# WGLab/DeepMod

Measured on AMD Instinct MI355X. Metric: base-positions/sec (whole node), E. coli 5mC wd21/f7 BiLSTM, higher is better.
Workload: dtype f16x3

## Files before the change

deepmod_amd/csrc/deepmod_hip.hip:

```cpp
#include "kernels.h"

#include <dlfcn.h>
#include <rccl/rccl.h>

#include <algorithm>
#include <cmath>
#include <cstdarg>
#include <cstdint>
#include <cstdio>
#include <cstring>
#include <string>
#include <utility>
#include <thread>
#include <type_traits>
#include <vector>

#include "../../include/deepmod_hip.h"
#include "head.hip.inc"

using dmk::Packed16;
using dmk::Packed32;

namespace {

// ... 292 lines not shown
    return ensure_pack(m->d_wpack16qi, dmk::pack_weights_f16q(m->host_weights.data(), true, m->i8s_q), dmk::f16q_prepare(1));
}


int launch_bilstm(dm_model* m, const float* d_x, long long xstride, int64_t n, float* d_prob, uint8_t* d_cls, const int* d_widx = nullptr) {
    if (n <= 0) return DM_OK;
    hipEvent_t e0 = nullptr, e1 = nullptr;
    if (m->profile) {
        if (m->events_used == m->events.size()) {
            if (m->events.size() >= 4096) {
                int rc = flush_profile(m);
                if (rc) return rc;
            } else {
                hipEvent_t a, b;
                HIP_TRY(hipEventCreate(&a));
                HIP_TRY(hipEventCreate(&b));
                m->events.emplace_back(a, b);
            }
        }
        e0 = m->events[m->events_used].first;
        e1 = m->events[m->events_used].second;
        ++m->events_used;
        HIP_TRY(hipEventRecord(e0, m->stream));
    }
    const int ntiles = int((n + dmk::TILE_M - 1) / dmk::TILE_M);
    {
        int rcp = ensure_plogit(m, ntiles);
        if (rcp) return rcp;
    }
    const long long npad = (long long)ntiles * dmk::TILE_M;
    int grid = std::min(2 * ntiles, m->grid_cap);
    if (2 * ntiles > m->grid_cap) {
        const int rounds = (2 * ntiles + m->grid_cap - 1) / m->grid_cap;
        grid = (2 * ntiles + rounds - 1) / rounds;
    }
    m->last_grid = grid;
    if (m->precision == DM_PREC_F16X3 || m->precision == DM_PREC_F16I8 || m->precision == DM_PREC_F16X3_ROLES) {
        const bool i8 = m->precision == DM_PREC_F16I8;
        const bool q16 = m->precision == DM_PREC_F16X3 && m->f16_q;
        const bool qi8 = i8 && m->f16_q;
#ifdef DM_WITH_F16S
        int rc = qi8 ? ensure_f16qi(m) : i8 ? ensure_f16i8(m) : (q16 ? ensure_f16q(m) : ensure_f16s(m));
#else
        if (!m->f16_q || m->precision == DM_PREC_F16X3_ROLES) return fail(DM_EINVAL, "the 32x32x16 kernels are not part of this build (tools/experiments/f16s: DM_WITH_F16S=1)");
        int rc = qi8 ? ensure_f16qi(m) : ensure_f16q(m);
#endif
        if (rc) return rc;
        dmk::F16Args a;
        a.wpack = qi8 ? m->d_wpack16qi : i8 ? m->d_wpack16i : q16 ? m->d_wpack16q : m->d_wpack16s;
        a.hpack = m->d_wout;
        a.x = d_x;
        a.xstride = xstride;
        a.widx = d_widx;
        a.n = n;
        a.ntiles = ntiles;
        a.plogit = m->d_plogit;
        a.len_shift = m->len_shift;
        a.range_flag = m->d_range_flag + m->range_cur;
        a.i8s = qi8 ? m->i8s_q : i8 ? m->i8s : nullptr;
        if (q16 || qi8) dmk::f16q_launch(qi8 ? 1 : 0, a, grid, m->stream);
#ifdef DM_WITH_F16S
        else dmk::f16s_launch(i8 ? 1 : (m->precision == DM_PREC_F16X3_ROLES ? 2 : 0), a, grid, m->stream);
#endif
    } else {
        dmk::F32Args a;
        a.wpack = m->d_wpack;
        a.bpack = m->d_bpack;
        a.hpack = m->d_hpack;
        a.bout0 = m->bout[0];
        a.bout1 = m->bout[1];
        a.x = d_x;
        a.xstride = xstride;
        a.widx = d_widx;
        a.n = n;
        a.prob = d_prob;
        a.cls = d_cls;
        a.scratch = m->d_scratch;
        a.ntiles = ntiles;
        a.dbg = m->d_dbg;
        a.dir_split = 1;
        a.plogit = m->d_plogit;
        dmk::f32_launch(a, grid, m->stream);
    }
    hipLaunchKernelGGL(lstmhead::head_finish_kernel, dim3(unsigned((n + 255) / 256)), dim3(256), 0, m->stream, m->d_plogit, (long long)n,
                       npad, m->bout[0], m->bout[1], d_prob, d_cls);
    HIP_TRY(hipGetLastError());
    if (m->profile) {
        HIP_TRY(hipEventRecord(e1, m->stream));
        ++m->prof_launches;
        m->prof_windows += n;
    }
    return DM_OK;
}

int range_error(dm_model* m) {
    return fail(DM_ERANGE, "DM_PREC_F16X3: an input feature is outside the representable range (features 0-5: |x| <= 65504, "
                "feature 6: |x| <= 65504 * 2^%d, no NaN); the results of these launches are invalid - repeat them with DM_PREC_F32",
                m->len_shift);
}
bool take_range_slot(dm_model* m, int slot) {
    volatile int* f = reinterpret_cast<volatile int*>(m->range_flag) + slot;
    const bool bad = *f != 0;
    *f = 0;
    return bad;
}
int check_range_all(dm_model* m) {
    if (!m->range_flag) return DM_OK;
    bool bad = take_range_slot(m, m->range_cur);
    for (int i = 0; i < DM_MARKS; ++i)
        if (m->mark_slot[i] >= 0) {
            bad |= take_range_slot(m, m->mark_slot[i]);
            m->slot_free[m->mark_slot[i]] = true;
            m->mark_slot[i] = -1;
        }
    for (int sl : m->range_orphans) {
        bad |= take_range_slot(m, sl);
        m->slot_free[sl] = true;
    }
    m->range_orphans.clear();
    return bad ? range_error(m) : DM_OK;
}
int sync_and_check(dm_model* m) {
    HIP_TRY(hipStreamSynchronize(m->stream));
    return check_range_all(m);
}

int predict_common(dm_model* m, const float* x, long long xstride, int64_t x_floats_total, int64_t n,
                   float* prob, uint8_t* cls, bool windows_materialised) {
    if (!m) return fail(DM_EINVAL, "null model");
    if (n < 0) return fail(DM_EINVAL, "negative window count");
    if (n == 0) return DM_OK;
    if (!x) return fail(DM_EINVAL, "null input");
    HIP_TRY(hipSetDevice(m->device));
    const bool xdev = is_device_ptr(x);
    const bool pdev = prob ? is_device_ptr(prob) : true;
    const bool cdev = cls ? is_device_ptr(cls) : true;
    if (xdev && pdev && cdev) {
        int rc = launch_bilstm(m, x, xstride, n, prob, cls);
        if (rc) return rc;
        if (!m->async) return sync_and_check(m);
        return DM_OK;
    }
    if (!windows_materialised) {
        int rc = ensure_stage(m, x_floats_total);
        if (rc) return rc;
        const float* dx = x;
        if (!xdev) {
            HIP_TRY(hipMemcpyAsync(m->d_x, x, sizeof(float) * x_floats_total, hipMemcpyHostToDevice, m->stream));
            dx = m->d_x;
        }
        for (int64_t off = 0; off < n; off += dm_model::STAGE_WINDOWS) {
            const int64_t cnt = std::min<int64_t>(dm_model::STAGE_WINDOWS, n - off);
            float* dp = prob ? (pdev ? prob + 2 * off : m->d_prob) : nullptr;
            uint8_t* dc = cls ? (cdev ? cls + off : m->d_cls) : nullptr;
            rc = launch_bilstm(m, dx + off * xstride, xstride, cnt, dp, dc);
            if (rc) return rc;
            if (prob && !pdev)
                HIP_TRY(hipMemcpyAsync(prob + 2 * off, m->d_prob, sizeof(float) * 2 * cnt, hipMemcpyDeviceToHost, m->stream));
            if (cls && !cdev) HIP_TRY(hipMemcpyAsync(cls + off, m->d_cls, cnt, hipMemcpyDeviceToHost, m->stream));
            rc = sync_and_check(m);
            if (rc) return rc;
        }
        return DM_OK;
    }
    const int64_t stage_floats = int64_t(dm_model::STAGE_WINDOWS) * DM_WINDOW * DM_NFEAT;
    int rc = ensure_stage(m, stage_floats);
    if (rc) return rc;
    if (!xdev && !m->d_x2) {
// ... 1093 lines not shown
```

deepmod_amd/csrc/kernels.h:

```cpp
#pragma once
#include <hip/hip_runtime.h>

#if defined(DM16Q_ABL_NOCELL) || defined(DM16Q_ABL_NODMA) || defined(DM16Q_ABL_MIX1) || defined(DM16Q_ABL_I8T) || defined(DM16Q_ABL_NOBAR) || defined(DM16Q_ABL_NOVMWAIT) || defined(DM16Q_AINIT) || defined(DM16Q_DEBUG_NOP) ||           \
    defined(DM16Q_NOCHUNK) || defined(DM16Q_NOPN) || defined(DM16Q_LOPACK) || defined(DM16Q_PRE) || defined(DM16Q_SNAKE) || defined(DM16Q_TRANS_COST) ||                     \
    defined(DM16S_ABL_2PROD) || defined(DM16S_ABL_B64) || defined(DM16S_ABL_LO_ONLY) || defined(DM16S_ABL_MFMA16) ||                              \
    defined(DM16S_ABL_MFMA16_PAD) || defined(DM16S_ABL_NOBAR) || defined(DM16S_ABL_NOCELL) || defined(DM16S_ABL_NODMA) ||                          \
    defined(DM16S_ABL_NOLDSA) || defined(DM16S_ADIST) || defined(DM16S_ALO_TRUNC) || defined(DM16S_PRE) || defined(DM_ABL_NOBAR) ||                \
    defined(DM_ABL_NODMA) || defined(DM_ABL_NOEPI) || defined(DM_ABL_NOSEQ) || defined(DM_TIMING) || defined(DM_TRACE) || defined(DM_TRACE2) ||   \
    defined(DM_WLO_TRUNC_ENV) || defined(DM_WLO_TRUNC_DEFAULT) || defined(DM_WITH_F16X3_ROLES) || defined(DM16R_DMA_M) ||                         \
    defined(DM_F16X3_SHAPE_DEFAULT) || defined(DM_WAVES) || defined(DM_MT) || defined(DM_WITH_F16S)
#define DM_ANY_EXPERIMENT_SWITCH 1
#ifndef DM_EXPERIMENT
#error "an ablation / experiment macro is defined without -DDM_EXPERIMENT: timing-only kernels must not be built into the product by a stray -D"
#endif
#else
#define DM_ANY_EXPERIMENT_SWITCH 0
#endif


#if defined(DM_WITH_F16X3_ROLES) && !defined(DM_WITH_F16S)
#error "the roles experiment lives in the translation unit of the 32x32x16 kernels: build it with -DDM_WITH_F16S as well"
#endif

#include <algorithm>
#include <cmath>
#include <cstdint>
#include <cstdlib>
#include <cstring>
#include <vector>

#include "../../include/deepmod_hip.h"

#ifndef DM_F16X3_SHAPE_DEFAULT
#define DM_F16X3_SHAPE_DEFAULT 16
#endif

namespace dmk {

constexpr int TILE_M = 128;

inline float gate_scale(int gc) { return (gc >= 100 && gc < 200) ? 2.8853900817779268f : -1.4426950408889634f; }


struct Packed32 {
    std::vector<float> w, b, h;
    float bout[2];
};

struct Packed16 {
    std::vector<unsigned char> w;
    float max_abs = 0.0f;
    bool finite = true;
    int len_shift = 0;
};

inline int choose_len_shift(const float* flat) {
    float m = 0.0f;
    const float* p = flat;
    for (int d = 0; d < 2; ++d) {
        const float* row = p + size_t(DM_NFEAT - 1) * 400;
        for (int gc = 0; gc < 400; ++gc) m = std::max(m, std::fabs(row[gc] * gate_scale(gc)));
        p += size_t(DM_NFEAT + DM_HIDDEN) * 400 + 400 + 2 * (size_t(2 * DM_HIDDEN) * 400 + 400);
    }
    int k = 10;
    while (k > 0 && !(m * std::ldexp(1.0f, k) <= 32768.0f)) --k;
    return k;
}



struct F16Args {
    const unsigned char* wpack;
    const float* hpack;
    const float* x;
    long long xstride;
    const int* widx;
    long long n;
    int ntiles;
    float* plogit;
    int len_shift;
    int* range_flag;
    const float* i8s;
};
struct F32Args {
    const float *wpack, *bpack, *hpack;
    float bout0, bout1;
    const float* x;
// ... 31 lines not shown
```

deepmod_amd/csrc/lstm_f16q.hip.inc:

```
#ifndef DM16Q_TRANS_COST
#define DM16Q_TRANS_COST 2
#endif
namespace lstm16q {

using lstmc::floatx2;
using lstmc::floatx4;
using lstmc::halfx2;
using lstmc::halfx8;
using lstmc::uintx4;
using lstmc::Params;
using lstmc::ex2;
using lstmc::rcp;
using lstmc::min60;
using lstmc::split_pack;
using lstmc::static_for;
using lstmc::as_h8;

constexpr int HID = 100, NFEAT = 7, WIN = 21, LIVE = 11;
constexpr int NTILE = 13;
constexpr int WAVES = 4, THREADS = 64 * WAVES, TILE_M = 32 * WAVES;
constexpr int KS_L0 = 4, KS_L12 = 7;
constexpr int REC_BYTES = 4096;
constexpr int MIX_BYTES = 2048;
constexpr int TILE_BYTES_L0 = (KS_L0 - 1) * REC_BYTES + 2 * MIX_BYTES, TILE_BYTES_L12 = (KS_L12 - 1) * REC_BYTES + MIX_BYTES;
constexpr int SLOT_BYTES = TILE_BYTES_L12;
constexpr int NSLOT = 2;
constexpr int C2_WAVE_BYTES = NTILE * 1024;
constexpr int C2_LAYER_BYTES = WAVES * C2_WAVE_BYTES;
constexpr size_t LDS_BYTES = size_t(NSLOT) * SLOT_BYTES + C2_LAYER_BYTES;
constexpr size_t LDS_BYTES_I8 = LDS_BYTES + C2_LAYER_BYTES;
constexpr size_t WEIGHT_BYTES_DIR = size_t(NTILE) * (TILE_BYTES_L0 + 2 * TILE_BYTES_L12);
constexpr size_t WEIGHT_BYTES = 2 * WEIGHT_BYTES_DIR;

using lstmc::intx4;
using lstmc::I8_MAGIC;
using lstmc::I8_HI_SCALE;
using lstmc::I8_LO_SCALE;
struct CellPipe {
    float ef[4], ei[4], ej[4], eo[4], t0[4], t1[4];
    unsigned hi01, hi23, lo01, lo23, i01, i23;
    floatx2 fold[2];
    floatx2 kmagic, khi, klo;
    static constexpr int NM = 14;
    template <int PRE, int FMT>
    __device__ static constexpr int nops(int M) {
        constexpr int n[9] = {12, 12, 12, 12, 8, 4, 4, 8, 6};
        if (M == 0) return PRE ? 16 : 0;
        if (M <= 9) return n[M - 1];
        if (M == 10) return FMT >= 1 ? 2 : 0;
        if (M == 11) return 4;
#if defined(DM16Q_LOPACK)
        if (M == 12) return FMT == 2 ? 2 : 0;
#else
        if (M == 12) return FMT != 1 ? 2 : 0;
#endif
        return FMT >= 1 ? 8 : 0;
    }
    template <int M, int J, int FMT = 0>
    __device__ __forceinline__ void op(floatx4 (&g)[4], const intx4 (&gi)[4], const floatx2 (&S)[2], float* c2, const bool only_a) {
        constexpr float K2 = 2.0f * 1.4426950408889634f;
        constexpr int q = J & 3, lv = J >> 2;
#define DM_PIN(X) asm volatile("" : "+v"(X))
        if constexpr (M == 0) {
            constexpr int k = J >> 1, c = k >> 1, pr = k & 1;
            if (only_a && (c & 1)) return;
            if constexpr ((J & 1) == 0) {
                fold[pr] = floatx2{(float)gi[c][2 * pr], (float)gi[c][2 * pr + 1]};
            } else {
                const floatx2 gp = __builtin_elementwise_fma(fold[pr], S[pr], floatx2{g[c][2 * pr], g[c][2 * pr + 1]});
                g[c][2 * pr] = gp[0];
                g[c][2 * pr + 1] = gp[1];
            }
            return;
        }
        if (only_a && (((M <= 8 || M == 11) && (q & 1)) || (M == 9 && lv == 0 && (q & 1)))) return;
        if constexpr (M == 1) {
            if constexpr (lv == 0) { t0[q] = min60(g[q][1]); DM_PIN(t0[q]); }
            else if constexpr (lv == 1) { ef[q] = ex2(g[q][2]); DM_PIN(ef[q]); }
            else { ei[q] = ex2(g[q][0]); DM_PIN(ei[q]); }
        } else if constexpr (M == 2) {
            if constexpr (lv == 0) { ej[q] = ex2(t0[q]); DM_PIN(ej[q]); }
            else if constexpr (lv == 1) { eo[q] = ex2(g[q][3]); DM_PIN(eo[q]); }
            else { ef[q] = 1.0f + ef[q]; DM_PIN(ef[q]); }
        } else if constexpr (M == 3) {
            if constexpr (lv == 0) { ef[q] = rcp(ef[q]); DM_PIN(ef[q]); }
            else if constexpr (lv == 1) { t1[q] = 1.0f + ej[q]; DM_PIN(t1[q]); }
            else { t0[q] = fmaf(ej[q], K2, -K2); DM_PIN(t0[q]); }
        } else if constexpr (M == 4) {
            if constexpr (lv == 0) { ei[q] = fmaf(ei[q], t1[q], t1[q]); DM_PIN(ei[q]); }
            else if constexpr (lv == 1) { eo[q] = 1.0f + eo[q]; DM_PIN(eo[q]); }
            else { ei[q] = rcp(ei[q]); DM_PIN(ei[q]); }
        } else if constexpr (M == 5) {
            if constexpr (lv == 0) { t0[q] = t0[q] * ei[q]; DM_PIN(t0[q]); }
            else { c2[q] = fmaf(c2[q], ef[q], t0[q]); DM_PIN(c2[q]); }
        } else if constexpr (M == 6) {
            { t0[q] = ex2(c2[q]); DM_PIN(t0[q]); }
        } else if constexpr (M == 7) {
            { t1[q] = t0[q] - 1.0f; DM_PIN(t1[q]); }
        } else if constexpr (M == 8) {
            if constexpr (lv == 0) { t0[q] = fmaf(t0[q], eo[q], eo[q]); DM_PIN(t0[q]); }
            else { t0[q] = rcp(t0[q]); DM_PIN(t0[q]); }
        } else if constexpr (M == 9) {
            if constexpr (lv == 0) { t1[q] = t1[q] * t0[q]; DM_PIN(t1[q]); }
            else if constexpr (J == 4) { hi01 = __builtin_bit_cast(unsigned, halfx2{(_Float16)t1[0], (_Float16)t1[1]}); DM_PIN(hi01); }
            else { hi23 = __builtin_bit_cast(unsigned, halfx2{(_Float16)t1[2], (_Float16)t1[3]}); DM_PIN(hi23); }
        } else if constexpr (M == 10) {
            const floatx2 v = __builtin_elementwise_fma(floatx2{t1[2 * J], t1[2 * J + 1]}, khi, kmagic);
            ef[2 * J] = v[0];
            ef[2 * J + 1] = v[1];
        } else if constexpr (M == 11) {
#if defined(DM16Q_LOPACK) && DM16Q_LOPACK == 1
            if constexpr (FMT == 0) {
                if constexpr (q == 0) asm volatile("v_fma_mixlo_f16 %0, %1, -1.0, %2 op_sel:[0,0,0] op_sel_hi:[1,0,0]" : "+v"(lo01) : "v"(hi01), "v"(t1[0]));
// ... 173 lines not shown
    intx4 acci[3][4];
    floatx2 i8s[3][2];
    CellPipe cp;
    float xf[2][2];
    int slot;
};

template <int LAYER, int MM>
__device__ __forceinline__ void c2_load(WaveState& w, const unsigned c2lds, const int tile, float (&row)[4]) {
    if constexpr (LAYER == 2) {
#pragma unroll
        for (int q = 0; q < 4; ++q) row[q] = w.c2reg[tile][q];
    } else if constexpr (LAYER == 1 && MM == 0) {
#pragma unroll
        for (int q = 0; q < 4; ++q) row[q] = w.c1reg[tile][q];
    } else {
        floatx4 v;
        asm volatile("ds_read_b128 %0, %1 offset:%2" : "=v"(v) : "v"(c2lds), "i"(LAYER * C2_LAYER_BYTES));
#pragma unroll
        for (int q = 0; q < 4; ++q) row[q] = v[q];
    }
}
template <int LAYER, int MM>
__device__ __forceinline__ void c2_store(WaveState& w, const unsigned c2lds, const int tile, const float (&row)[4]) {
    if constexpr (LAYER == 2) {
#pragma unroll
        for (int q = 0; q < 4; ++q) w.c2reg[tile][q] = row[q];
    } else if constexpr (LAYER == 1 && MM == 0) {
#pragma unroll
        for (int q = 0; q < 4; ++q) w.c1reg[tile][q] = row[q];
    } else {
        asm volatile("ds_write_b128 %0, %1 offset:%2" :: "v"(c2lds), "v"(floatx4{row[0], row[1], row[2], row[3]}), "i"(LAYER * C2_LAYER_BYTES) : "memory");
    }
}

__device__ __forceinline__ unsigned lo_lo(unsigned a, unsigned b) { return __builtin_amdgcn_perm(b, a, 0x05040100u); }
__device__ __forceinline__ unsigned hi_lo(unsigned a, unsigned b) { return __builtin_amdgcn_alignbit(b, a, 16); }

template <int LAYER, bool FIRST, int MM>
__device__ __forceinline__ void run_stage(const Params& p, WaveState& w, const unsigned lds_base, const unsigned c2_wave, const unsigned char* wdir, const int dir, const int s,
                                          const float* xwin0, const float* xwin1, const int wave_s, const unsigned lane16, const int grp, const unsigned one2) {
    using K = StageKind<LAYER, FIRST>;
    constexpr bool L0 = K::L0;
    constexpr int KS = K::KS;
    constexpr int PREV = (LAYER + 2) % 3;
    constexpr int I8 = (MM == 1 && !(L0 && FIRST)) ? 1 : 0;
    constexpr int PRE = I8;
    constexpr int PPRE = (MM == 1 && !(PREV == 0 && FIRST)) ? 1 : 0;
    constexpr int FMT = MM == 0 ? 0 : (LAYER == 2 ? 2 : 1);
    constexpr size_t LAYER_OFF[3] = {0, size_t(NTILE) * TILE_BYTES_L0, size_t(NTILE) * (TILE_BYTES_L0 + TILE_BYTES_L12)};
    uintx4 (&own)[12] = w.own[LAYER];
    const uintx4 (&inp)[12] = w.own[L0 ? 0 : LAYER - 1];
    const floatx2 (&S)[2] = w.i8s[LAYER];
    const floatx2 (&PS)[2] = w.i8s[PREV];
    uintx4 mx[2], mx2[2];
    unsigned x0p[2] = {0u, 0u}, x1a[2] = {0u, 0u}, x1b[2] = {0u, 0u};
    if constexpr (L0) {
        bool bad = false;
#pragma unroll
        for (int hh = 0; hh < 2; ++hh) {
            float v0 = w.xf[hh][0], v1 = w.xf[hh][1];
            bad |= !(fabsf(v0) <= 65504.0f);
            if (grp < 2) bad |= !(fabsf(v1) <= 65504.0f);
            else {
                const float t = rintf(v1 * p.len_scale);
                bad |= !(fabsf(t) <= 65504.0f);
                v1 = grp == 2 ? v1 - t * p.len_mul : t;
            }
            unsigned xh, xl;
            split_pack(v0, v1, xh, xl);
            x0p[hh] = lo_lo(xh, xl);
            x1a[hh] = __builtin_amdgcn_perm(xh, xh, 0x03020302u);
            x1b[hh] = __builtin_amdgcn_perm(xl, xl, 0x03020302u);
        }
        if (bad) *p.range_flag = 1;
        if (s + 1 < LIVE) {
            const int row = dir == 0 ? s + 1 : WIN - 2 - s;
            const int f1 = 4 + grp < NFEAT ? 4 + grp : NFEAT - 1;
            w.xf[0][0] = xwin0[row * NFEAT + grp]; w.xf[0][1] = xwin0[row * NFEAT + f1];
            w.xf[1][0] = xwin1[row * NFEAT + grp]; w.xf[1][1] = xwin1[row * NFEAT + f1];
        }
    }
    const bool last_stage = LAYER == 2 && s == LIVE - 1;
    static_for<NTILE>([&](auto Tc) {
        constexpr int T = decltype(Tc)::value;
        constexpr int P = T == 0 ? NTILE - 1 : T - 1;
        constexpr int accT = T == NTILE - 1 ? 2 : (T & 1), accP = P == NTILE - 1 ? 2 : (P & 1);
        constexpr bool WITH_B = T < NTILE - 1;
        constexpr int NMF = (WITH_B ? 4 : 2) * (I8 ? 2 : 3);
        float c2row[4];
        if constexpr (T == 0) c2_load<PREV, MM>(w, c2_wave + unsigned(NTILE - 1) * 1024u, NTILE - 1, c2row);
        else c2_load<LAYER, MM>(w, c2_wave + unsigned(P) * 1024u, P, c2row);
        const unsigned a_addr = lds_base + unsigned(w.slot) * SLOT_BYTES + lane16;
#ifdef DM16Q_AINIT
        AQuad a[2] = {};
#else
        AQuad a[2];
#endif
        load_a<K::rec_off(0), WITH_B, K::mixed(0)>(a[0], a_addr);
        if (!(last_stage && T == NTILE - 1)) {
            if constexpr (T + 1 < NTILE) {
                unsigned toff = unsigned(T + 1) * K::TILE_BYTES;
                asm volatile("" : "+s"(toff));
                stage_tile<K::DMA_BYTES>(wdir + (LAYER_OFF[LAYER] + K::DMA_OFF) + toff, lds_base + unsigned(w.slot ^ 1) * SLOT_BYTES + K::DMA_OFF, wave_s, lane16);
            } else {
                using KN = StageKind<(LAYER + 1) % 3, FIRST && LAYER < 2>;
                stage_tile<KN::DMA_BYTES>(wdir + (LAYER_OFF[(LAYER + 1) % 3] + KN::DMA_OFF), lds_base + unsigned(w.slot ^ 1) * SLOT_BYTES + KN::DMA_OFF, wave_s, lane16);
            }
        }
        floatx4 (&d)[4] = w.acc[accT];
        intx4 (&di)[4] = w.acci[accT];
        floatx4 (&g)[4] = w.acc[accP];
        const intx4 (&gi)[4] = w.acci[accP];
        const floatx4 z4 = {0.f, 0.f, 0.f, 0.f};
        const intx4 zi4 = {0, 0, 0, 0};
        constexpr int NCH = DM16Q_PRE + NMF * (KS - 1);
#ifdef DM16Q_NOCHUNK
#define DM_CHUNK(C) do { if constexpr ((C) == NCH - 1) { if constexpr (T == 0) w.cp.template all<PPRE, 0>(g, gi, PS, c2row, true); else w.cp.template all<PRE, FMT>(g, gi, S, c2row, false); } } while (0)
#else
#define DM_CHUNK(C) do { if constexpr (T == 0) w.cp.template chunk<(C), NCH, PPRE, 0>(g, gi, PS, c2row, true); else w.cp.template chunk<(C), NCH, PRE, FMT>(g, gi, S, c2row, false); } while (0)
#endif
        if constexpr (KS > 1) static_for<DM16Q_PRE>([&](auto cc) { DM_CHUNK(decltype(cc)::value); });
        static_for<KS>([&](auto ic) {
            constexpr int i = decltype(ic)::value;
            constexpr int MIXED = K::mixed(i);
            if constexpr (i + 1 < KS) load_a<K::rec_off(i + 1), WITH_B, K::mixed(i + 1)>(a[(i + 1) & 1], a_addr);
            if constexpr (i == KS - 1) {
                if constexpr (KS == 1) {
                    if constexpr (T == 0) w.cp.template all<PPRE, 0>(g, gi, PS, c2row, true);
                    else w.cp.template all<PRE, FMT>(g, gi, S, c2row, false);
                }
#ifdef DM16Q_ABL_NOCELL
                w.cp.hi01 = w.cp.hi23 = 0x2E662E66u; w.cp.lo01 = w.cp.lo23 = 0x0A660A66u;
#endif
                if constexpr (T == 0) {
                    w.m12[PREV][0][0] = lo_lo(w.cp.hi01, w.cp.hi01); w.m12[PREV][0][1] = lo_lo(w.cp.hi01, w.cp.lo01);
                    w.m12[PREV][1][0] = lo_lo(w.cp.hi23, w.cp.hi23); w.m12[PREV][1][1] = lo_lo(w.cp.hi23, w.cp.lo23);
                    c2_store<PREV, MM>(w, c2_wave + unsigned(NTILE - 1) * 1024u, NTILE - 1, c2row);
                } else {
                    constexpr int pt = P >> 2, pr = P & 3;
                    unsigned s01, s23;
                    if constexpr (FMT == 0) { s01 = w.cp.lo01; s23 = w.cp.lo23; }
                    else if constexpr (FMT == 1) { s01 = w.cp.i01; s23 = w.cp.i23; }
                    else { s01 = last_stage ? w.cp.lo01 : w.cp.i01; s23 = last_stage ? w.cp.lo23 : w.cp.i23; }
                    w.nxt[quad(pt, 0, 0)][pr] = w.cp.hi01; w.nxt[quad(pt, 0, 1)][pr] = s01;
                    w.nxt[quad(pt, 1, 0)][pr] = w.cp.hi23; w.nxt[quad(pt, 1, 1)][pr] = s23;
                    c2_store<LAYER, MM>(w, c2_wave + unsigned(P) * 1024u, P, c2row);
                }
            }
            if constexpr (T == 0) {
                static_for<3>([&](auto pc) {
                    constexpr int pt = decltype(pc)::value;
                    if constexpr (KS > 3 ? pt == i : i == 0) {
#pragma unroll
                        for (int e = 0; e < 4; ++e) w.own[PREV][4 * pt + e] = w.nxt[4 * pt + e];
                    }
                });
            }
            if constexpr (MIXED != 0 && T == 0) {
#pragma unroll
                for (int hh = 0; hh < 2; ++hh) {
                    unsigned in_hl;
                    if constexpr (L0) in_hl = x0p[hh];
                    else in_hl = w.m12[LAYER - 1][hh][1];
                    unsigned own_hh = w.m12[LAYER][hh][0], own_hl = w.m12[LAYER][hh][1];
                    asm volatile("" : "+v"(own_hh), "+v"(own_hl), "+v"(in_hl));
                    mx[hh] = uintx4{own_hh, hi_lo(own_hl, in_hl), in_hl, one2};
                    if constexpr (L0) mx2[hh] = uintx4{x1a[hh], x1b[hh], 0u, 0u};
                }
            }
            wait_a<(i + 1 < KS ? a_reads(WITH_B, K::mixed(i + 1 < KS ? i + 1 : i)) : 0)>(a[i & 1]);
            constexpr int C0 = DM16Q_PRE + NMF * i;
#define DM_MF(AOP, BOP, Q, NO)                                                                                              \
            d[Q] = __builtin_amdgcn_mfma_f32_16x16x32_f16(AOP, BOP, (i == 0 && (NO) == 0) ? z4 : d[Q], 0, 0, 0);              \
            asm volatile(DM16Q_AFTER_MFMA : "+v"(d[Q]) : "v"(AOP), "v"(BOP));
#define DM_MI(AOP, BOP, Q)                                                                                                  \
            di[Q] = __builtin_amdgcn_mfma_i32_16x16x64_i8(__builtin_bit_cast(intx4, AOP), __builtin_bit_cast(intx4, BOP), i == 0 ? zi4 : di[Q], 0, 0, 0); \
            asm volatile(DM16Q_AFTER_MFMA : "+v"(di[Q]) : "v"(AOP), "v"(BOP));
#define DM_CELLQ(N_) if constexpr (KS > 1 && i < KS - 1) DM_CHUNK(C0 + (N_))
            if constexpr (MIXED != 0) {
                const halfx8 b0 = as_h8(mx[0]), b1 = as_h8(mx[1]);
                DM_MF(a[i & 1].hiA, b0, 0, 0)
                DM_MF(a[i & 1].hiA, b1, 2, 0)
                if constexpr (WITH_B) { DM_MF(a[i & 1].hiB, b0, 1, 0) DM_MF(a[i & 1].hiB, b1, 3, 0) }
                if constexpr (MIXED == 2) {
                    const halfx8 e0 = as_h8(mx2[0]), e1 = as_h8(mx2[1]);
                    DM_MF(a[i & 1].loA, e0, 0, 1)
                    DM_MF(a[i & 1].loA, e1, 2, 1)
                    if constexpr (WITH_B) { DM_MF(a[i & 1].loB, e0, 1, 1) DM_MF(a[i & 1].loB, e1, 3, 1) }
                }
            } else {
                constexpr int t = K::opnd(i);
                halfx8 bh[2], bl[2];
#pragma unroll
                for (int hh = 0; hh < 2; ++hh) {
                    if constexpr (K::is_own(i)) { bh[hh] = as_h8(own[quad(t, hh, 0)]); bl[hh] = as_h8(own[quad(t, hh, 1)]); }
                    else { bh[hh] = as_h8(inp[quad(t, hh, 0)]); bl[hh] = as_h8(inp[quad(t, hh, 1)]); }
                }
                if constexpr (I8) {
                    DM_MF(a[i & 1].hiA, bh[0], 0, 0) DM_CELLQ(0);
                    DM_MF(a[i & 1].hiA, bh[1], 2, 0) DM_CELLQ(1);
                    if constexpr (WITH_B) { DM_MF(a[i & 1].hiB, bh[0], 1, 0) DM_CELLQ(2); DM_MF(a[i & 1].hiB, bh[1], 3, 0) DM_CELLQ(3); }
                    DM_MI(a[i & 1].loA, bl[0], 0) DM_CELLQ(WITH_B ? 4 : 2);
                    DM_MI(a[i & 1].loA, bl[1], 2) DM_CELLQ(WITH_B ? 5 : 3);
                    if constexpr (WITH_B) { DM_MI(a[i & 1].loB, bl[0], 1) DM_CELLQ(6); DM_MI(a[i & 1].loB, bl[1], 3) DM_CELLQ(7); }
                } else {
#ifdef DM16Q_SNAKE
                DM_MF(a[i & 1].hiA, bh[0], 0, 0) DM_CELLQ(0);
                if constexpr (WITH_B) { DM_MF(a[i & 1].hiB, bh[0], 1, 0) DM_CELLQ(1); DM_MF(a[i & 1].hiB, bh[1], 3, 0) DM_CELLQ(2); }
                DM_MF(a[i & 1].hiA, bh[1], 2, 0) DM_CELLQ(WITH_B ? 3 : 1);
                DM_MF(a[i & 1].loA, bh[1], 2, 1) DM_CELLQ(WITH_B ? 4 : 2);
                if constexpr (WITH_B) { DM_MF(a[i & 1].loB, bh[1], 3, 1) DM_CELLQ(5); DM_MF(a[i & 1].loB, bh[0], 1, 1) DM_CELLQ(6); }
                DM_MF(a[i & 1].loA, bh[0], 0, 1) DM_CELLQ(WITH_B ? 7 : 3);
                DM_MF(a[i & 1].hiA, bl[0], 0, 2) DM_CELLQ(WITH_B ? 8 : 4);
                if constexpr (WITH_B) { DM_MF(a[i & 1].hiB, bl[0], 1, 2) DM_CELLQ(9); DM_MF(a[i & 1].hiB, bl[1], 3, 2) DM_CELLQ(10); }
                DM_MF(a[i & 1].hiA, bl[1], 2, 2) DM_CELLQ(WITH_B ? 11 : 5);
#else
                DM_MF(a[i & 1].hiA, bh[0], 0, 0) DM_CELLQ(0);
                DM_MF(a[i & 1].hiA, bh[1], 2, 0) DM_CELLQ(1);
                if constexpr (WITH_B) { DM_MF(a[i & 1].hiB, bh[0], 1, 0) DM_CELLQ(2); DM_MF(a[i & 1].hiB, bh[1], 3, 0) DM_CELLQ(3); }
#ifdef DM16Q_ABL_I8T
                DM_MI(a[i & 1].loA, bl[0], 0) DM_CELLQ(WITH_B ? 4 : 2); DM_CELLQ(WITH_B ? 5 : 3);
                DM_MI(a[i & 1].loA, bl[1], 2) DM_CELLQ(WITH_B ? 6 : 4); DM_CELLQ(WITH_B ? 7 : 5);
                if constexpr (WITH_B) { DM_MI(a[i & 1].loB, bl[0], 1) DM_CELLQ(8); DM_CELLQ(9); DM_MI(a[i & 1].loB, bl[1], 3) DM_CELLQ(10); DM_CELLQ(11); }
#else
                DM_MF(a[i & 1].loA, bh[0], 0, 1) DM_CELLQ(WITH_B ? 4 : 2);
                DM_MF(a[i & 1].loA, bh[1], 2, 1) DM_CELLQ(WITH_B ? 5 : 3);
                if constexpr (WITH_B) { DM_MF(a[i & 1].loB, bh[0], 1, 1) DM_CELLQ(6); DM_MF(a[i & 1].loB, bh[1], 3, 1) DM_CELLQ(7); }
                DM_MF(a[i & 1].hiA, bl[0], 0, 2) DM_CELLQ(WITH_B ? 8 : 4);
                DM_MF(a[i & 1].hiA, bl[1], 2, 2) DM_CELLQ(WITH_B ? 9 : 5);
                if constexpr (WITH_B) { DM_MF(a[i & 1].hiB, bl[0], 1, 2) DM_CELLQ(10); DM_MF(a[i & 1].hiB, bl[1], 3, 2) DM_CELLQ(11); }
#endif
#endif
                }
            }
#undef DM_MF
#undef DM_MI
#undef DM_CELLQ
        });
#undef DM_CHUNK
#ifndef DM16Q_ABL_NOVMWAIT
        asm volatile("s_waitcnt vmcnt(0)" ::: "memory");
#endif
#ifndef DM16Q_ABL_NOBAR
        __builtin_amdgcn_s_barrier();
#endif
        w.slot ^= 1;
    });
}

template <int MM>
__global__ __launch_bounds__(THREADS, 1) void bilstm_f16q_kernel(const Params p) {
    extern __shared__ __attribute__((aligned(16))) unsigned char lds16q[];
    const int lane = threadIdx.x & 63;
    const int wave = threadIdx.x >> 6;
    const int wave_s = __builtin_amdgcn_readfirstlane(wave);
    const int grp = lane >> 4, n16 = lane & 15;
    const unsigned lane16 = unsigned(lane) * 16u;
    const unsigned lds_base = (unsigned)(size_t)lds16q;
    const unsigned c2_wave = lds_base + unsigned(NSLOT) * SLOT_BYTES + unsigned(wave) * C2_WAVE_BYTES + lane16;
    const unsigned one2 = grp == 0 ? 0x3C003C00u : 0u;
    const int nwork = 2 * p.ntiles;
    for (int work = blockIdx.x; work < nwork; work += gridDim.x) {
        const int tile = work >> 1, dir = work & 1;
        const long long tile0 = (long long)tile * TILE_M;
        const long long w_out = tile0 + wave * 32 + n16;
        long long wi0 = w_out, wi1 = w_out + 16;
        if (wi0 > p.n - 1) wi0 = p.n - 1;
        if (wi1 > p.n - 1) wi1 = p.n - 1;
        const float* xwin0 = p.x + (p.widx ? (long long)p.widx[wi0] : wi0) * p.xstride;
        const float* xwin1 = p.x + (p.widx ? (long long)p.widx[wi1] : wi1) * p.xstride;
        const unsigned char* wdir = p.wpack + size_t(dir) * WEIGHT_BYTES_DIR;

        WaveState w;
#pragma unroll
        for (int l = 0; l < 3; ++l) {
#pragma unroll
            for (int q = 0; q < 12; ++q) w.own[l][q] = uintx4{0u, 0u, 0u, 0u};
#pragma unroll
            for (int hh = 0; hh < 2; ++hh) w.m12[l][hh][0] = w.m12[l][hh][1] = 0u;
        }
#pragma unroll
        for (int q = 0; q < 12; ++q) w.nxt[q] = uintx4{0u, 0u, 0u, 0u};
#pragma unroll
        for (int t = 0; t < NTILE; ++t)
#pragma unroll
            for (int q = 0; q < 4; ++q) w.c2reg[t][q] = w.c1reg[t][q] = 0.0f;
#pragma unroll
        for (int t = 0; t < 3; ++t)
#pragma unroll
            for (int q = 0; q < 4; ++q) w.acc[t][q] = floatx4{0.f, 0.f, 0.f, 0.f};
        w.cp.hi01 = w.cp.hi23 = w.cp.lo01 = w.cp.lo23 = 0u;
        if constexpr (MM == 1) {
#pragma unroll
            for (int t = 0; t < 3; ++t)
#pragma unroll
                for (int q = 0; q < 4; ++q) w.acci[t][q] = intx4{0, 0, 0, 0};
#pragma unroll
            for (int l = 0; l < 3; ++l)
#pragma unroll
                for (int k = 0; k < 2; ++k) w.i8s[l][k] = floatx2{p.i8s[(dir * 3 + l) * 4 + 2 * k], p.i8s[(dir * 3 + l) * 4 + 2 * k + 1]};
            w.cp.kmagic = floatx2{I8_MAGIC, I8_MAGIC};
            w.cp.khi = floatx2{I8_HI_SCALE, I8_HI_SCALE};
            w.cp.klo = floatx2{I8_LO_SCALE, I8_LO_SCALE};
            w.cp.i01 = w.cp.i23 = 0u;
        }
        w.slot = 0;
        __syncthreads();
        {
            const floatx4 z4 = {0.f, 0.f, 0.f, 0.f};
#pragma unroll
            for (int t = 0; t < NTILE; ++t) {
                asm volatile("ds_write_b128 %0, %1" :: "v"(c2_wave + unsigned(t * 1024)), "v"(z4) : "memory");
                if constexpr (MM == 1) asm volatile("ds_write_b128 %0, %1 offset:%2" :: "v"(c2_wave + unsigned(t * 1024)), "v"(z4), "i"(C2_LAYER_BYTES) : "memory");
            }
        }
        {
            using K0 = StageKind<0, true>;
            stage_tile<K0::DMA_BYTES>(wdir + K0::DMA_OFF, lds_base + K0::DMA_OFF, wave_s, lane16);
        }
        {
            const int row = dir == 0 ? 0 : WIN - 1;
            const int f1 = 4 + grp < NFEAT ? 4 + grp : NFEAT - 1;
            w.xf[0][0] = xwin0[row * NFEAT + grp]; w.xf[0][1] = xwin0[row * NFEAT + f1];
            w.xf[1][0] = xwin1[row * NFEAT + grp]; w.xf[1][1] = xwin1[row * NFEAT + f1];
        }
        asm volatile("s_waitcnt vmcnt(0) lgkmcnt(0)" ::: "memory");
        __syncthreads();

#define DM_STAGE(LAYER, FIRST, S_) run_stage<LAYER, FIRST, MM>(p, w, lds_base, c2_wave, wdir, dir, S_, xwin0, xwin1, wave_s, lane16, grp, one2)
        DM_STAGE(0, true, 0);
        DM_STAGE(1, true, 0);
        DM_STAGE(2, true, 0);
        for (int s = 1; s < LIVE; ++s) {
            DM_STAGE(0, false, s);
            DM_STAGE(1, false, s);
            DM_STAGE(2, false, s);
        }
#undef DM_STAGE
        {
            float c2row[4];
#pragma unroll
            for (int q = 0; q < 4; ++q) c2row[q] = w.c2reg[NTILE - 1][q];
            w.cp.template all<MM, 0>(w.acc[2], w.acci[2], w.i8s[2], c2row, true);
            w.m12[2][0][1] = lo_lo(w.cp.hi01, w.cp.lo01);
            w.m12[2][1][1] = lo_lo(w.cp.hi23, w.cp.lo23);
#pragma unroll
            for (int q = 0; q < 12; ++q) w.own[2][q] = w.nxt[q];
        }
#pragma unroll
        for (int hh = 0; hh < 2; ++hh) {
            float hsum0 = 0.0f, hsum1 = 0.0f;
            static_for<NTILE>([&](auto Sc) {
                constexpr int S = decltype(Sc)::value;
                unsigned hi, lo;
                if constexpr (S < 12) { hi = w.own[2][quad(S >> 2, hh, 0)][S & 3]; lo = w.own[2][quad(S >> 2, hh, 1)][S & 3]; }
                else { hi = w.m12[2][hh][1]; lo = w.m12[2][hh][1] >> 16; }
                const halfx2 h2 = __builtin_bit_cast(halfx2, hi), l2 = __builtin_bit_cast(halfx2, lo);
#pragma unroll
                for (int rh = 0; rh < (S < 12 ? 2 : 1); ++rh) {
                    const float h = (float)h2[rh] + (float)l2[rh];
                    const float* wo = p.hpack + (dir * HID + 8 * S + 4 * rh + grp) * 2;
                    hsum0 = fmaf(h, wo[0], hsum0);
                    hsum1 = fmaf(h, wo[1], hsum1);
                }
            });
            hsum0 += __shfl_xor(hsum0, 16, 64);
            hsum1 += __shfl_xor(hsum1, 16, 64);
            hsum0 += __shfl_xor(hsum0, 32, 64);
            hsum1 += __shfl_xor(hsum1, 32, 64);
            if (lane < 16) {
                float* pl = p.plogit + (size_t(dir) * p.ntiles * TILE_M + size_t(w_out + 16 * hh)) * 2;
                pl[0] = hsum0;
                pl[1] = hsum1;
            }
        }
    }
}

}
```

Before: 48.43 million.

## Use four-slot LDS weight ring with paired barriers and cross-tile A prefetch

For the non-int8 f16q kernel, the LDS weight staging ring grows from two to four slots. DMA now prefetches two tiles ahead, and the vmcnt wait plus workgroup barrier run only every other tile. The first A-operand load of each odd tile's successor is issued during the last k-step, which hides LDS latency across tile boundaries. This costs more LDS (two extra slots) and more complex slot indexing. It also drops the SNAKE/I8T ablation variants and adopts the snake MFMA order as the default, and adds ablation switches (PAIRBAR, NOHEAD).

```diff
diff --git a/deepmod_amd/csrc/deepmod_hip.hip b/deepmod_amd/csrc/deepmod_hip.hip
--- a/deepmod_amd/csrc/deepmod_hip.hip
+++ b/deepmod_amd/csrc/deepmod_hip.hip
@@ -398,8 +398,10 @@
         a.plogit = m->d_plogit;
         dmk::f32_launch(a, grid, m->stream);
     }
+#ifndef DM_ABL_NOHEAD
     hipLaunchKernelGGL(lstmhead::head_finish_kernel, dim3(unsigned((n + 255) / 256)), dim3(256), 0, m->stream, m->d_plogit, (long long)n,
                        npad, m->bout[0], m->bout[1], d_prob, d_cls);
+#endif
     HIP_TRY(hipGetLastError());
     if (m->profile) {
         HIP_TRY(hipEventRecord(e1, m->stream));
diff --git a/deepmod_amd/csrc/kernels.h b/deepmod_amd/csrc/kernels.h
--- a/deepmod_amd/csrc/kernels.h
+++ b/deepmod_amd/csrc/kernels.h
@@ -1,8 +1,8 @@
 #pragma once
 #include <hip/hip_runtime.h>
 
-#if defined(DM16Q_ABL_NOCELL) || defined(DM16Q_ABL_NODMA) || defined(DM16Q_ABL_MIX1) || defined(DM16Q_ABL_I8T) || defined(DM16Q_ABL_NOBAR) || defined(DM16Q_ABL_NOVMWAIT) || defined(DM16Q_AINIT) || defined(DM16Q_DEBUG_NOP) ||           \
-    defined(DM16Q_NOCHUNK) || defined(DM16Q_NOPN) || defined(DM16Q_LOPACK) || defined(DM16Q_PRE) || defined(DM16Q_SNAKE) || defined(DM16Q_TRANS_COST) ||                     \
+#if defined(DM16Q_ABL_NOCELL) || defined(DM16Q_ABL_NODMA) || defined(DM16Q_ABL_MIX1) || defined(DM16Q_ABL_PAIRBAR) || defined(DM16Q_ABL_NOBAR) || defined(DM16Q_ABL_NOVMWAIT) || defined(DM16Q_AINIT) || defined(DM16Q_DEBUG_NOP) ||           \
+    defined(DM16Q_NOCHUNK) || defined(DM16Q_NOPN) || defined(DM16Q_LOPACK) || defined(DM16Q_PRE) || defined(DM_ABL_NOHEAD) || defined(DM16Q_TRANS_COST) ||                     \
     defined(DM16S_ABL_2PROD) || defined(DM16S_ABL_B64) || defined(DM16S_ABL_LO_ONLY) || defined(DM16S_ABL_MFMA16) ||                              \
     defined(DM16S_ABL_MFMA16_PAD) || defined(DM16S_ABL_NOBAR) || defined(DM16S_ABL_NOCELL) || defined(DM16S_ABL_NODMA) ||                          \
     defined(DM16S_ABL_NOLDSA) || defined(DM16S_ADIST) || defined(DM16S_ALO_TRUNC) || defined(DM16S_PRE) || defined(DM_ABL_NOBAR) ||                \
diff --git a/deepmod_amd/csrc/lstm_f16q.hip.inc b/deepmod_amd/csrc/lstm_f16q.hip.inc
--- a/deepmod_amd/csrc/lstm_f16q.hip.inc
+++ b/deepmod_amd/csrc/lstm_f16q.hip.inc
@@ -24,11 +24,17 @@
 constexpr int MIX_BYTES = 2048;
 constexpr int TILE_BYTES_L0 = (KS_L0 - 1) * REC_BYTES + 2 * MIX_BYTES, TILE_BYTES_L12 = (KS_L12 - 1) * REC_BYTES + MIX_BYTES;
 constexpr int SLOT_BYTES = TILE_BYTES_L12;
-constexpr int NSLOT = 2;
+__host__ __device__ constexpr int ring_slots(int mm) {
+#ifdef DM16Q_ABL_PAIRBAR
+    return 2;
+#else
+    return mm == 0 ? 4 : 2;
+#endif
+}
 constexpr int C2_WAVE_BYTES = NTILE * 1024;
 constexpr int C2_LAYER_BYTES = WAVES * C2_WAVE_BYTES;
-constexpr size_t LDS_BYTES = size_t(NSLOT) * SLOT_BYTES + C2_LAYER_BYTES;
-constexpr size_t LDS_BYTES_I8 = LDS_BYTES + C2_LAYER_BYTES;
+constexpr size_t LDS_BYTES = size_t(ring_slots(0)) * SLOT_BYTES + C2_LAYER_BYTES;
+constexpr size_t LDS_BYTES_I8 = size_t(ring_slots(1)) * SLOT_BYTES + 2 * C2_LAYER_BYTES;
 constexpr size_t WEIGHT_BYTES_DIR = size_t(NTILE) * (TILE_BYTES_L0 + 2 * TILE_BYTES_L12);
 constexpr size_t WEIGHT_BYTES = 2 * WEIGHT_BYTES_DIR;
 
@@ -368,6 +374,11 @@
         }
     }
     const bool last_stage = LAYER == 2 && s == LIVE - 1;
+#ifdef DM16Q_AINIT
+    AQuad a[2] = {};
+#else
+    AQuad a[2];
+#endif
     static_for<NTILE>([&](auto Tc) {
         constexpr int T = decltype(Tc)::value;
         constexpr int P = T == 0 ? NTILE - 1 : T - 1;
@@ -378,21 +389,20 @@
         if constexpr (T == 0) c2_load<PREV, MM>(w, c2_wave + unsigned(NTILE - 1) * 1024u, NTILE - 1, c2row);
         else c2_load<LAYER, MM>(w, c2_wave + unsigned(P) * 1024u, P, c2row);
         const unsigned a_addr = lds_base + unsigned(w.slot) * SLOT_BYTES + lane16;
-#ifdef DM16Q_AINIT
-        AQuad a[2] = {};
-#else
-        AQuad a[2];
-#endif
-        load_a<K::rec_off(0), WITH_B, K::mixed(0)>(a[0], a_addr);
-        if (!(last_stage && T == NTILE - 1)) {
-            if constexpr (T + 1 < NTILE) {
-                unsigned toff = unsigned(T + 1) * K::TILE_BYTES;
-                asm volatile("" : "+s"(toff));
-                stage_tile<K::DMA_BYTES>(wdir + (LAYER_OFF[LAYER] + K::DMA_OFF) + toff, lds_base + unsigned(w.slot ^ 1) * SLOT_BYTES + K::DMA_OFF, wave_s, lane16);
-            } else {
-                using KN = StageKind<(LAYER + 1) % 3, FIRST && LAYER < 2>;
-                stage_tile<KN::DMA_BYTES>(wdir + (LAYER_OFF[(LAYER + 1) % 3] + KN::DMA_OFF), lds_base + unsigned(w.slot ^ 1) * SLOT_BYTES + KN::DMA_OFF, wave_s, lane16);
-            }
+        constexpr int NS = ring_slots(MM);
+        constexpr bool EDGE = NS == 2 || (T & 1) == 0;
+        constexpr bool PF_OUT = NS == 4 && (T & 1) == 1, PF_IN = NS == 4 && T >= 2 && (T & 1) == 0;
+        constexpr int AOFS = PF_IN ? (KS & 1) : 0;
+        if constexpr (!PF_IN) load_a<K::rec_off(0), WITH_B, K::mixed(0)>(a[0], a_addr);
+        constexpr int AHEAD = NS / 2;
+        if constexpr (T + AHEAD < NTILE) {
+            unsigned toff = unsigned(T + AHEAD) * K::TILE_BYTES;
+            asm volatile("" : "+s"(toff));
+            stage_tile<K::DMA_BYTES>(wdir + (LAYER_OFF[LAYER] + K::DMA_OFF) + toff, lds_base + unsigned((w.slot + AHEAD) & (NS - 1)) * SLOT_BYTES + K::DMA_OFF, wave_s, lane16);
+        } else if (!last_stage) {
+            using KN = StageKind<(LAYER + 1) % 3, FIRST && LAYER < 2>;
+            constexpr size_t noff = size_t(T + AHEAD - NTILE) * KN::TILE_BYTES;
+            stage_tile<KN::DMA_BYTES>(wdir + (LAYER_OFF[(LAYER + 1) % 3] + KN::DMA_OFF + noff), lds_base + unsigned((w.slot + AHEAD) & (NS - 1)) * SLOT_BYTES + KN::DMA_OFF, wave_s, lane16);
         }
         floatx4 (&d)[4] = w.acc[accT];
         intx4 (&di)[4] = w.acci[accT];
@@ -410,7 +420,8 @@
         static_for<KS>([&](auto ic) {
             constexpr int i = decltype(ic)::value;
             constexpr int MIXED = K::mixed(i);
-            if constexpr (i + 1 < KS) load_a<K::rec_off(i + 1), WITH_B, K::mixed(i + 1)>(a[(i + 1) & 1], a_addr);
+            AQuad& ai = a[(i + AOFS) & 1];
+            if constexpr (i + 1 < KS) load_a<K::rec_off(i + 1), WITH_B, K::mixed(i + 1)>(a[(i + 1 + AOFS) & 1], a_addr);
             if constexpr (i == KS - 1) {
                 if constexpr (KS == 1) {
                     if constexpr (T == 0) w.cp.template all<PPRE, 0>(g, gi, PS, c2row, true);
@@ -455,7 +466,9 @@
                     if constexpr (L0) mx2[hh] = uintx4{x1a[hh], x1b[hh], 0u, 0u};
                 }
             }
-            wait_a<(i + 1 < KS ? a_reads(WITH_B, K::mixed(i + 1 < KS ? i + 1 : i)) : 0)>(a[i & 1]);
+            constexpr bool WITH_B_NEXT = T + 1 < NTILE - 1;
+            if constexpr (PF_OUT && i == KS - 1) load_a<K::rec_off(0), WITH_B_NEXT, K::mixed(0)>(a[KS & 1], lds_base + unsigned((w.slot + 1) & (NS - 1)) * SLOT_BYTES + lane16);
+            wait_a<(i + 1 < KS ? a_reads(WITH_B, K::mixed(i + 1 < KS ? i + 1 : i)) : (PF_OUT ? a_reads(WITH_B_NEXT, K::mixed(0)) : 0))>(ai);
             constexpr int C0 = DM16Q_PRE + NMF * i;
 #define DM_MF(AOP, BOP, Q, NO)                                                                                              \
             d[Q] = __builtin_amdgcn_mfma_f32_16x16x32_f16(AOP, BOP, (i == 0 && (NO) == 0) ? z4 : d[Q], 0, 0, 0);              \
@@ -466,14 +479,14 @@
 #define DM_CELLQ(N_) if constexpr (KS > 1 && i < KS - 1) DM_CHUNK(C0 + (N_))
             if constexpr (MIXED != 0) {
                 const halfx8 b0 = as_h8(mx[0]), b1 = as_h8(mx[1]);
-                DM_MF(a[i & 1].hiA, b0, 0, 0)
-                DM_MF(a[i & 1].hiA, b1, 2, 0)
-                if constexpr (WITH_B) { DM_MF(a[i & 1].hiB, b0, 1, 0) DM_MF(a[i & 1].hiB, b1, 3, 0) }
+                DM_MF(ai.hiA, b0, 0, 0)
+                DM_MF(ai.hiA, b1, 2, 0)
+                if constexpr (WITH_B) { DM_MF(ai.hiB, b0, 1, 0) DM_MF(ai.hiB, b1, 3, 0) }
                 if constexpr (MIXED == 2) {
                     const halfx8 e0 = as_h8(mx2[0]), e1 = as_h8(mx2[1]);
-                    DM_MF(a[i & 1].loA, e0, 0, 1)
-                    DM_MF(a[i & 1].loA, e1, 2, 1)
-                    if constexpr (WITH_B) { DM_MF(a[i & 1].loB, e0, 1, 1) DM_MF(a[i & 1].loB, e1, 3, 1) }
+                    DM_MF(ai.loA, e0, 0, 1)
+                    DM_MF(ai.loA, e1, 2, 1)
+                    if constexpr (WITH_B) { DM_MF(ai.loB, e0, 1, 1) DM_MF(ai.loB, e1, 3, 1) }
                 }
             } else {
                 constexpr int t = K::opnd(i);
@@ -484,40 +497,22 @@
                     else { bh[hh] = as_h8(inp[quad(t, hh, 0)]); bl[hh] = as_h8(inp[quad(t, hh, 1)]); }
                 }
                 if constexpr (I8) {
-                    DM_MF(a[i & 1].hiA, bh[0], 0, 0) DM_CELLQ(0);
-                    DM_MF(a[i & 1].hiA, bh[1], 2, 0) DM_CELLQ(1);
-                    if constexpr (WITH_B) { DM_MF(a[i & 1].hiB, bh[0], 1, 0) DM_CELLQ(2); DM_MF(a[i & 1].hiB, bh[1], 3, 0) DM_CELLQ(3); }
-                    DM_MI(a[i & 1].loA, bl[0], 0) DM_CELLQ(WITH_B ? 4 : 2);
-                    DM_MI(a[i & 1].loA, bl[1], 2) DM_CELLQ(WITH_B ? 5 : 3);
-                    if constexpr (WITH_B) { DM_MI(a[i & 1].loB, bl[0], 1) DM_CELLQ(6); DM_MI(a[i & 1].loB, bl[1], 3) DM_CELLQ(7); }
+                    DM_MF(ai.hiA, bh[0], 0, 0) DM_CELLQ(0);
+                    DM_MF(ai.hiA, bh[1], 2, 0) DM_CELLQ(1);
+                    if constexpr (WITH_B) { DM_MF(ai.hiB, bh[0], 1, 0) DM_CELLQ(2); DM_MF(ai.hiB, bh[1], 3, 0) DM_CELLQ(3); }
+                    DM_MI(ai.loA, bl[0], 0) DM_CELLQ(WITH_B ? 4 : 2);
+                    DM_MI(ai.loA, bl[1], 2) DM_CELLQ(WITH_B ? 5 : 3);
+                    if constexpr (WITH_B) { DM_MI(ai.loB, bl[0], 1) DM_CELLQ(6); DM_MI(ai.loB, bl[1], 3) DM_CELLQ(7); }
                 } else {
-#ifdef DM16Q_SNAKE
-                DM_MF(a[i & 1].hiA, bh[0], 0, 0) DM_CELLQ(0);
-                if constexpr (WITH_B) { DM_MF(a[i & 1].hiB, bh[0], 1, 0) DM_CELLQ(1); DM_MF(a[i & 1].hiB, bh[1], 3, 0) DM_CELLQ(2); }
-                DM_MF(a[i & 1].hiA, bh[1], 2, 0) DM_CELLQ(WITH_B ? 3 : 1);
-                DM_MF(a[i & 1].loA, bh[1], 2, 1) DM_CELLQ(WITH_B ? 4 : 2);
-                if constexpr (WITH_B) { DM_MF(a[i & 1].loB, bh[1], 3, 1) DM_CELLQ(5); DM_MF(a[i & 1].loB, bh[0], 1, 1) DM_CELLQ(6); }
-                DM_MF(a[i & 1].loA, bh[0], 0, 1) DM_CELLQ(WITH_B ? 7 : 3);
-                DM_MF(a[i & 1].hiA, bl[0], 0, 2) DM_CELLQ(WITH_B ? 8 : 4);
-                if constexpr (WITH_B) { DM_MF(a[i & 1].hiB, bl[0], 1, 2) DM_CELLQ(9); DM_MF(a[i & 1].hiB, bl[1], 3, 2) DM_CELLQ(10); }
-                DM_MF(a[i & 1].hiA, bl[1], 2, 2) DM_CELLQ(WITH_B ? 11 : 5);
-#else
-                DM_MF(a[i & 1].hiA, bh[0], 0, 0) DM_CELLQ(0);
-                DM_MF(a[i & 1].hiA, bh[1], 2, 0) DM_CELLQ(1);
-                if constexpr (WITH_B) { DM_MF(a[i & 1].hiB, bh[0], 1, 0) DM_CELLQ(2); DM_MF(a[i & 1].hiB, bh[1], 3, 0) DM_CELLQ(3); }
-#ifdef DM16Q_ABL_I8T
-                DM_MI(a[i & 1].loA, bl[0], 0) DM_CELLQ(WITH_B ? 4 : 2); DM_CELLQ(WITH_B ? 5 : 3);
-                DM_MI(a[i & 1].loA, bl[1], 2) DM_CELLQ(WITH_B ? 6 : 4); DM_CELLQ(WITH_B ? 7 : 5);
-                if constexpr (WITH_B) { DM_MI(a[i & 1].loB, bl[0], 1) DM_CELLQ(8); DM_CELLQ(9); DM_MI(a[i & 1].loB, bl[1], 3) DM_CELLQ(10); DM_CELLQ(11); }
-#else
-                DM_MF(a[i & 1].loA, bh[0], 0, 1) DM_CELLQ(WITH_B ? 4 : 2);
-                DM_MF(a[i & 1].loA, bh[1], 2, 1) DM_CELLQ(WITH_B ? 5 : 3);
-                if constexpr (WITH_B) { DM_MF(a[i & 1].loB, bh[0], 1, 1) DM_CELLQ(6); DM_MF(a[i & 1].loB, bh[1], 3, 1) DM_CELLQ(7); }
-                DM_MF(a[i & 1].hiA, bl[0], 0, 2) DM_CELLQ(WITH_B ? 8 : 4);
-                DM_MF(a[i & 1].hiA, bl[1], 2, 2) DM_CELLQ(WITH_B ? 9 : 5);
-                if constexpr (WITH_B) { DM_MF(a[i & 1].hiB, bl[0], 1, 2) DM_CELLQ(10); DM_MF(a[i & 1].hiB, bl[1], 3, 2) DM_CELLQ(11); }
-#endif
-#endif
+                DM_MF(ai.hiA, bh[0], 0, 0) DM_CELLQ(0);
+                if constexpr (WITH_B) { DM_MF(ai.hiB, bh[0], 1, 0) DM_CELLQ(1); DM_MF(ai.hiB, bh[1], 3, 0) DM_CELLQ(2); }
+                DM_MF(ai.hiA, bh[1], 2, 0) DM_CELLQ(WITH_B ? 3 : 1);
+                DM_MF(ai.loA, bh[1], 2, 1) DM_CELLQ(WITH_B ? 4 : 2);
+                if constexpr (WITH_B) { DM_MF(ai.loB, bh[1], 3, 1) DM_CELLQ(5); DM_MF(ai.loB, bh[0], 1, 1) DM_CELLQ(6); }
+                DM_MF(ai.loA, bh[0], 0, 1) DM_CELLQ(WITH_B ? 7 : 3);
+                DM_MF(ai.hiA, bl[0], 0, 2) DM_CELLQ(WITH_B ? 8 : 4);
+                if constexpr (WITH_B) { DM_MF(ai.hiB, bl[0], 1, 2) DM_CELLQ(9); DM_MF(ai.hiB, bl[1], 3, 2) DM_CELLQ(10); }
+                DM_MF(ai.hiA, bl[1], 2, 2) DM_CELLQ(WITH_B ? 11 : 5);
                 }
             }
 #undef DM_MF
@@ -525,13 +520,19 @@
 #undef DM_CELLQ
         });
 #undef DM_CHUNK
+#ifdef DM16Q_ABL_PAIRBAR
+        if constexpr ((T & 1) == 0) {
+#else
+        if constexpr (EDGE) {
+#endif
 #ifndef DM16Q_ABL_NOVMWAIT
         asm volatile("s_waitcnt vmcnt(0)" ::: "memory");
 #endif
 #ifndef DM16Q_ABL_NOBAR
         __builtin_amdgcn_s_barrier();
 #endif
-        w.slot ^= 1;
+        }
+        w.slot = (w.slot + 1) & (NS - 1);
     });
 }
 
@@ -544,7 +545,7 @@
     const int grp = lane >> 4, n16 = lane & 15;
     const unsigned lane16 = unsigned(lane) * 16u;
     const unsigned lds_base = (unsigned)(size_t)lds16q;
-    const unsigned c2_wave = lds_base + unsigned(NSLOT) * SLOT_BYTES + unsigned(wave) * C2_WAVE_BYTES + lane16;
+    const unsigned c2_wave = lds_base + unsigned(ring_slots(MM)) * SLOT_BYTES + unsigned(wave) * C2_WAVE_BYTES + lane16;
     const unsigned one2 = grp == 0 ? 0x3C003C00u : 0u;
     const int nwork = 2 * p.ntiles;
     for (int work = blockIdx.x; work < nwork; work += gridDim.x) {
@@ -604,6 +605,7 @@
         {
             using K0 = StageKind<0, true>;
             stage_tile<K0::DMA_BYTES>(wdir + K0::DMA_OFF, lds_base + K0::DMA_OFF, wave_s, lane16);
+            if constexpr (ring_slots(MM) == 4) stage_tile<K0::DMA_BYTES>(wdir + (K0::TILE_BYTES + K0::DMA_OFF), lds_base + (SLOT_BYTES + K0::DMA_OFF), wave_s, lane16);
         }
         {
             const int row = dir == 0 ? 0 : WIN - 1;
```

Result: faster. 49.36 million (median of 6 runs) (+1.9%).
